# worxli/ORB_SLAM

Hardware: AMD Instinct MI355X
Metric: frames/sec ORB extract+match (640x480, 1000 kp) (higher is better)
Workload: dtype u8

## Files before the change

orb_slam_amd/csrc/orbx_extract.hip:

```cpp
#include <algorithm>
#include <type_traits>

#include "orbx_device.h"
#include "orbx_internal.h"

namespace orbx {

constexpr size_t kRetainLds = 128 * 1024;
constexpr int kRetainCellCap = 512;
constexpr int kSplitMinFrames = 16;
constexpr size_t kResizeLds = 96 * 1024;

__constant__ __attribute__((aligned(4))) int8_t c_pattern[256][4] = {
#include "orbx_pattern.inc"
};

#ifdef ORBX_FAST_PROFILE
__device__ unsigned long long g_fast_prof[16];
__device__ inline unsigned long long fp_stamp()
{
    unsigned long long t;
    asm volatile("s_memtime %0\n\ts_waitcnt lgkmcnt(0)" : "=s"(t)::"memory");
    return t;
}
#define FP_T0() unsigned long long _ft = fp_stamp()
#define FP_MARK(k)                                                                  \
    do {                                                                            \
        const unsigned long long _n = fp_stamp();                                   \
        if (threadIdx.x == 0) atomicAdd(&g_fast_prof[k], _n - _ft);                 \
        _ft = _n;                                                                   \
    } while (0)
#define FP_ADD(k, v) atomicAdd(&g_fast_prof[k], (unsigned long long)(v))
extern "C" int orbx_debug_fast_prof(unsigned long long* out)
{
    return hipMemcpyFromSymbol(out, HIP_SYMBOL(g_fast_prof), sizeof(unsigned long long) * 16) == hipSuccess ? 0 : -2;
}
#else
#define FP_T0()
#define FP_MARK(k)
#define FP_ADD(k, v)
#endif

struct ExtractArgs {
    const LevelGeom* levels;
    const CellGeom* cells;
    const ResizeCol* res_cols;
    const ResizeRow* res_rows;
    const int* umax;
    const uint8_t* frames;
    uint8_t* pyr_raw;
    uint8_t* pyr_blur;
    uint32_t* cell_lists;
    int32_t* cell_count;
    uint32_t* level_keys;
    int32_t* level_count;
    orbx_keypoint* out_kps;
    uint8_t* out_desc;
    int32_t* out_n;
    int32_t* error_flags;
    uint8_t* host_out;
    int32_t* retain_scratch;
    uint64_t* cell_keys64;
    uint64_t* level_keys64;
    int harris;
    int fp_contract;
    int nth_pivot;
    long long frame_pyr_bytes;
    int first_slot;
    int w, h;
    int nlevels, ncells, list_entries, level_entries, nfeatures;
    int fast_th, fast_th_low;
    int max_list_cap, max_level_cap;
    int l0_direct;
};

struct LevelSrc {
    const uint8_t* base;
    int stride;
};
static_assert(kEdge % 16 == 0, "the direct level 0 keeps the padded level's 16-byte alignment");
__device__ __forceinline__ LevelSrc level_src(const ExtractArgs& a, int f, int level, long long off, int stride)
{
    if (a.l0_direct && level == 0)
        return {a.frames + ((long long)(a.first_slot + f) * a.w * a.h - (long long)kEdge * a.w - kEdge), a.w};
    return {a.pyr_raw + (size_t)f * a.frame_pyr_bytes + off, stride};
}

template <class T>
__device__ __forceinline__ T cget(const T* p, int i)
{
#if defined(__HIP_DEVICE_COMPILE__)
    return ((const __attribute__((address_space(4))) T*)p)[i];
#else
    return p[i];
#endif
}

__device__ inline uint8_t sat_u8(int v) { return (uint8_t)min(max(v, 0), 255); }
__device__ inline int sat_s16(int v) { return min(max(v, -32768), 32767); }

struct RowWalk {
    int r, q, dr, dq, nq;
    __device__ RowWalk(int start, int stride, int n_q) : nq(n_q)
    {
        r = start / n_q;
        q = start - r * n_q;
        dr = stride / n_q;
        dq = stride - dr * n_q;
    }
    __device__ void next()
    {
        r += dr;
        q += dq;
        if (q >= nq) {
            q -= nq;
            r++;
        }
    }
};


template <int kBatch, typename T, typename Load>
__device__ inline void stage_to_lds(T* dst, int n, int tid, int nthr, Load load)
{
    for (int u0 = 0; u0 < n; u0 += kBatch * nthr) {
        T v[kBatch];
#pragma unroll
        for (int k = 0; k < kBatch; k++) v[k] = load(min(u0 + k * nthr + tid, n - 1));
#pragma unroll
        for (int k = 0; k < kBatch; k++) dst[min(u0 + k * nthr + tid, n - 1)] = v[k];
    }
}

constexpr int kPyrRows = 8;
constexpr int kPyr0Shift = (16 - kEdge % 16) % 16;

__global__ __launch_bounds__(256) void k_pyr_level0(ExtractArgs a, int q_lo, int nint)
{
    const int f = blockIdx.y;
    const LevelGeom L = cget(a.levels, 0);
    const int qpr = L.stride >> 4, nstrips = (L.ph + kPyrRows - 1) / kPyrRows;
    const int nbord = qpr - nint;
    int idx = blockIdx.x * blockDim.x + threadIdx.x;
    const uint8_t* src = a.frames + (size_t)(a.first_slot + f) * a.w * a.h;
    uint8_t* dst = a.pyr_raw + (size_t)f * a.frame_pyr_bytes + L.off;
    if (idx < nint * nstrips) {
        const int strip = idx / nint, q = q_lo + (idx - strip * nint), px0 = 16 * q;
        const int al = px0 - kEdge - kPyr0Shift;
        const int py_first = strip * kPyrRows;
        uint4 lo[kPyrRows], hi[kPyrRows];
#pragma unroll
        for (int rr = 0; rr < kPyrRows; rr++) {
            const int py = min(py_first + rr, L.ph - 1);
            const uint8_t* row = src + (size_t)reflect101(py - kEdge, L.h) * a.w + al;
            lo[rr] = *reinterpret_cast<const uint4*>(row);
            hi[rr] = *reinterpret_cast<const uint4*>(row + 16);
        }
#pragma unroll
        for (int rr = 0; rr < kPyrRows; rr++) {
            const uint32_t w[8] = {lo[rr].x, lo[rr].y, lo[rr].z, lo[rr].w, hi[rr].x, hi[rr].y, hi[rr].z, hi[rr].w};
            constexpr int d = kPyr0Shift >> 2, b = kPyr0Shift & 3;
            uint32_t o[4];
#pragma unroll
            for (int k = 0; k < 4; k++)
                o[k] = b ? __builtin_amdgcn_alignbyte(w[k + d + 1], w[k + d], b) : w[k + d];
            if (py_first + rr < L.ph)
                *reinterpret_cast<uint4*>(dst + (size_t)(py_first + rr) * L.stride + px0) = make_uint4(o[0], o[1], o[2], o[3]);
        }
        return;
    }
    idx -= nint * nstrips;
    if (idx >= nbord * L.ph) return;
    const int py = idx / nbord, k = idx - py * nbord;
    const int q = k < q_lo ? k : k + nint, px0 = 16 * q;
    const uint8_t* row = src + (size_t)reflect101(py - kEdge, L.h) * a.w;
    if (kEdge == 16 && a.w % 16 == 0 && a.w >= 32) {
        const int w16 = a.w >> 4;
        uint4 v = make_uint4(0, 0, 0, 0);
        if (q == 0) {
            const uint4 A = *reinterpret_cast<const uint4*>(row), B = *reinterpret_cast<const uint4*>(row + 16);
            v.x = __builtin_amdgcn_perm(B.x, A.w, 0x01020304u);
            v.y = __builtin_amdgcn_perm(A.w, A.z, 0x01020304u);
            v.z = __builtin_amdgcn_perm(A.z, A.y, 0x01020304u);
            v.w = __builtin_amdgcn_perm(A.y, A.x, 0x01020304u);
        } else if (q <= w16) {
            v = *reinterpret_cast<const uint4*>(row + 16 * (q - 1));
        } else if (q == w16 + 1) {
            const uint4 A = *reinterpret_cast<const uint4*>(row + a.w - 32), B = *reinterpret_cast<const uint4*>(row + a.w - 16);
            v.x = __builtin_amdgcn_perm(B.w, B.z, 0x03040506u);
            v.y = __builtin_amdgcn_perm(B.z, B.y, 0x03040506u);
            v.z = __builtin_amdgcn_perm(B.y, B.x, 0x03040506u);
            v.w = __builtin_amdgcn_perm(B.x, A.w, 0x03040506u);
        }
        *reinterpret_cast<uint4*>(dst + (size_t)py * L.stride + px0) = v;
        return;
    }
    uint8_t v[16];
#pragma unroll
    for (int i = 0; i < 16; i++) v[i] = px0 + i < L.pw ? row[reflect101(px0 + i - kEdge, L.w)] : 0;
    uint32_t o[4];
#pragma unroll
    for (int i = 0; i < 4; i++)
        o[i] = v[4 * i] | (uint32_t)v[4 * i + 1] << 8 | (uint32_t)v[4 * i + 2] << 16 | (uint32_t)v[4 * i + 3] << 24;
    *reinterpret_cast<uint4*>(dst + (size_t)py * L.stride + px0) = make_uint4(o[0], o[1], o[2], o[3]);
}

__device__ inline uint8_t resize_pixel(const uint8_t* prev, int pstride, const ResizeCol& c,
                                       const ResizeRow& r, bool vec)
{
    const uint8_t* r0 = prev + (size_t)r.sy0 * pstride;
    const uint8_t* r1 = prev + (size_t)r.sy1 * pstride;
    const int S0 = r0[c.sx0] * c.a0 + r0[c.sx1] * c.a1;
    const int S1 = r1[c.sx0] * c.a0 + r1[c.sx1] * c.a1;
    if (vec) {
        const int x0 = sat_s16(S0 >> 4), y0 = sat_s16(S1 >> 4);
        int v = sat_s16(((x0 * r.b0) >> 16) + ((y0 * r.b1) >> 16));
        v = sat_s16(v + 2) >> 2;
        return sat_u8(v);
    }
    return sat_u8((S0 * r.b0 + S1 * r.b1 + (1 << 21)) >> 22);
}

__global__ __launch_bounds__(256) void k_pyr_resize(ExtractArgs a, int level)
{
    const int f = blockIdx.y;
    const LevelGeom L = cget(a.levels, level);
    const LevelGeom P = cget(a.levels, level - 1);
    const int wpr = L.stride >> 2, nstrips = (L.ph + kPyrRows - 1) / kPyrRows;
    const int idx = blockIdx.x * blockDim.x + threadIdx.x;
    if (idx >= wpr * nstrips) return;
    const int strip = idx / wpr, q = idx - strip * wpr, px0 = 4 * q;
    const LevelSrc ps = level_src(a, f, level - 1, P.off, P.stride);
    const uint8_t* prev = ps.base + (size_t)kEdge * ps.stride + kEdge;
    uint8_t* dst = a.pyr_raw + (size_t)f * a.frame_pyr_bytes + L.off;
    ResizeCol c[4];
    bool vec[4], on[4];
#pragma unroll
    for (int b = 0; b < 4; b++) {
        on[b] = px0 + b < L.pw;
        const int x = on[b] ? reflect101(px0 + b - kEdge, L.w) : 0;
        c[b] = a.res_cols[L.res_col_off + x];
        vec[b] = x < L.nvec_resize;
    }
#pragma unroll
    for (int rr = 0; rr < kPyrRows; rr++) {
        const int py = min(strip * kPyrRows + rr, L.ph - 1);
        const ResizeRow r = a.res_rows[L.res_row_off + reflect101(py - kEdge, L.h)];
        uint32_t word = 0;
#pragma unroll
        for (int b = 0; b < 4; b++)
            if (on[b]) word |= (uint32_t)resize_pixel(prev, ps.stride, c[b], r, vec[b]) << (8 * b);
        if (strip * kPyrRows + rr < L.ph) *reinterpret_cast<uint32_t*>(dst + (size_t)py * L.stride + px0) = word;
    }
}

struct ResizeLevel {
    long long off, poff;
    int stride, pstride, w, h, pw, ph, ph_parent_h, nvec, span, strip_off, row_off, col_off;
    int packed;
    int plevel, ppad;
};

__global__ __launch_bounds__(256) void k_pyr_resize_lds(ExtractArgs a, ResizeLevel L, int pitch)
{
    extern __shared__ uint4 s_dyn[];
    __shared__ ResizeRow s_rows[kResRows];
    const int f = blockIdx.y, tid = threadIdx.x;
    const int py0 = blockIdx.x * kResRows, nrows = min(kResRows, L.ph - py0);
    const int nch = pitch >> 4;
    ResizeCol* s_cols = reinterpret_cast<ResizeCol*>(s_dyn + (size_t)L.span * nch);
    uint8_t* s_src = reinterpret_cast<uint8_t*>(s_dyn);
    const int lo = a.res_rows[L.strip_off + blockIdx.x].sy0;
    if (tid < nrows) s_rows[tid] = a.res_rows[L.row_off + reflect101(py0 + tid - kEdge, L.h)];
    stage_to_lds<4>(s_cols, L.w, tid, (int)blockDim.x, [&](int x) { return a.res_cols[L.col_off + x]; });
    const int nsrc = min(L.span, L.ph_parent_h - lo);
    const LevelSrc ps = level_src(a, f, L.plevel, L.poff, L.pstride);
    const uint8_t* pbase = ps.base + (size_t)(lo + kEdge) * ps.stride + (kEdge - L.ppad);
#ifndef RES_NO_STAGE
    {
        const float inv = 1.0f / (float)nch;
        stage_to_lds<8>(s_dyn, nsrc * nch, tid, (int)blockDim.x, [&](int u) {
            const int r = (int)(((float)u + 0.5f) * inv), c = u - r * nch;
            return *reinterpret_cast<const uint4*>(pbase + (size_t)r * ps.stride + 16 * c);
        });
    }
#endif
    __syncthreads();
    uint8_t* dst = a.pyr_raw + (size_t)f * a.frame_pyr_bytes + L.off + (size_t)py0 * L.stride;
#ifdef RES_NO_COMPUTE
    if (tid < 64) reinterpret_cast<uint32_t*>(dst)[tid] = s_src[tid * 7];
    return;
#endif
    const int nq = L.stride >> 2;
    const int q_lo = (kEdge + 3) >> 2, q_hi = L.packed ? max(q_lo, (kEdge + min(L.w, L.nvec)) >> 2) : q_lo;
    const int nfast = q_hi - q_lo;
    typedef unsigned short orbx_us2 __attribute__((ext_vector_type(2)));
    auto mh = [](uint32_t x, uint32_t y) {
        return (uint32_t)(((unsigned long long)(x & 0xFFFFFFu) * (unsigned long long)(y & 0xFFFFFFu)) >> 32);
    };
    for (int t = tid; t < nfast; t += blockDim.x) {
        const int q = q_lo + t, x0 = 4 * q - kEdge;
        int ca[4];
        uint32_t sel[4], wgt[4];
#pragma unroll
        for (int b = 0; b < 4; b++) {
            const ResizeCol c = s_cols[x0 + b];
            ca[b] = L.ppad + c.sx0;
            wgt[b] = (uint32_t)(16 * c.a0) | (uint32_t)(16 * c.a1) << 16;
        }
        const int qa = ca[0] & ~3, sh = ca[0] & 3;
#pragma unroll
        for (int b = 0; b < 4; b++) {
            const uint32_t r = (uint32_t)(ca[b] - ca[0]);
            sel[b] = r | 0x0C00u | (r + 1) << 16 | 0x0C000000u;
        }
        auto hrow = [&](int sy, uint32_t (&S)[4]) {
            const uint32_t* d = reinterpret_cast<const uint32_t*>(s_src + (sy - lo) * pitch + qa);
            const uint32_t d0 = d[0], d1 = d[1], d2 = d[2];
            const uint32_t w0 = __builtin_amdgcn_alignbyte(d1, d0, sh), w1 = __builtin_amdgcn_alignbyte(d2, d1, sh);
#pragma unroll
            for (int b = 0; b < 4; b++)
                S[b] = __builtin_amdgcn_udot2(__builtin_bit_cast(orbx_us2, __builtin_amdgcn_perm(w1, w0, sel[b])),
                                              __builtin_bit_cast(orbx_us2, wgt[b]), 0u, false) &
                       0x00FFFF00u;
        };
        uint32_t H0[4], H1[4];
        int c0 = -1, c1 = -1;
        uint2 nxt = reinterpret_cast<const uint2*>(s_rows)[0];
        for (int rr = 0; rr < nrows; rr++) {
            const uint2 cur = nxt;
            if (rr + 1 < nrows) nxt = reinterpret_cast<const uint2*>(s_rows)[rr + 1];
            const uint32_t w0 = __builtin_amdgcn_readfirstlane(cur.x), w1 = __builtin_amdgcn_readfirstlane(cur.y);
            const int sy0 = (int)(int16_t)(w0 & 0xFFFF), sy1 = (int)(int16_t)(w0 >> 16);
            const uint32_t B0 = (w1 & 0xFFFFu) << 8, B1 = (w1 >> 16) << 8;
            uint32_t A[4], B[4];
            if (sy0 == c1) {
#pragma unroll
                for (int b = 0; b < 4; b++) A[b] = H1[b];
            } else if (sy0 == c0) {
#pragma unroll
                for (int b = 0; b < 4; b++) A[b] = H0[b];
            } else {
                hrow(sy0, A);
            }
            if (sy1 == sy0) {
#pragma unroll
                for (int b = 0; b < 4; b++) B[b] = A[b];
            } else if (sy1 == c1) {
#pragma unroll
                for (int b = 0; b < 4; b++) B[b] = H1[b];
            } else {
                hrow(sy1, B);
            }
#pragma unroll
            for (int b = 0; b < 4; b++) {
                H0[b] = A[b];
                H1[b] = B[b];
            }
            c0 = sy0;
            c1 = sy1;
            uint32_t word = 0;
#pragma unroll
            for (int b = 0; b < 4; b++) word |= ((mh(A[b], B0) + mh(B[b], B1) + 2) >> 2) << (8 * b);
            *reinterpret_cast<uint32_t*>(dst + (size_t)rr * L.stride + 4 * q) = word;
        }
    }
    const int nslow = nq - nfast;
    for (int item = tid; item < nrows * nslow; item += blockDim.x) {
        const int rr = item / nslow, k = item - rr * nslow;
        const int q = k < q_lo ? k : k + nfast, px0 = 4 * q;
        const ResizeRow R = s_rows[rr];
        uint32_t word = 0;
#pragma unroll
        for (int b = 0; b < 4; b++) {
            if (px0 + b >= L.pw) continue;
            const int x = reflect101(px0 + b - kEdge, L.w);
            const ResizeCol c = s_cols[x];
            const uint8_t* r0 = s_src + (R.sy0 - lo) * pitch + L.ppad + c.sx0;
            const uint8_t* r1 = s_src + (R.sy1 - lo) * pitch + L.ppad + c.sx0;
            const int S0 = r0[0] * c.a0 + r0[1] * c.a1, S1 = r1[0] * c.a0 + r1[1] * c.a1;
            int v;
            if (x < L.nvec)
                v = (((S0 >> 4) * R.b0 >> 16) + ((S1 >> 4) * R.b1 >> 16) + 2) >> 2;
            else
                v = (S0 * R.b0 + S1 * R.b1 + (1 << 21)) >> 22;
            word |= (uint32_t)sat_u8(v) << (8 * b);
        }
        *reinterpret_cast<uint32_t*>(dst + (size_t)rr * L.stride + px0) = word;
    }
}

#ifndef ORBX_CASCADE_SINGLE_THREADS
#define ORBX_CASCADE_SINGLE_THREADS 1024
#endif
#ifdef ORBX_CASC_PROFILE
__device__ unsigned long long g_casc_prof[kMaxLevels][4];
#define CASC_T0() unsigned long long _ct = __builtin_readcyclecounter()
#define CASC_MARK(l, k)                                                          \
    do {                                                                         \
        const unsigned long long _n = __builtin_readcyclecounter();              \
        if (blockIdx.x == 0 && threadIdx.x == 0) g_casc_prof[l][k] += _n - _ct;  \
        _ct = _n;                                                                \
    } while (0)
extern "C" int orbx_debug_casc_prof(unsigned long long* out)
{
    return hipMemcpyFromSymbol(out, HIP_SYMBOL(g_casc_prof), sizeof(g_casc_prof)) == hipSuccess ? 0 : -2;
}
#else
#define CASC_T0()
#define CASC_MARK(l, k)
#endif
template <int T>
__global__ __launch_bounds__(T) void k_pyr_cascade(ExtractArgs a, const int4* plan, int buf_x, int tab_off,
                                                   int tab_cols)
{
    CASC_T0();
    const bool kTab = T >= 1024 && tab_off > 0;
    extern __shared__ uint4 s_dyn[];
    uint8_t* const lds = reinterpret_cast<uint8_t*>(s_dyn);
    const int band = blockIdx.x, f = blockIdx.y, tid = threadIdx.x;
    uint8_t* pyr = a.pyr_raw + (size_t)f * a.frame_pyr_bytes;
    const uint8_t* img = a.frames + (size_t)(a.first_slot + f) * a.w * a.h;
    ResizeCol* const t_cols = reinterpret_cast<ResizeCol*>(lds + tab_off);
    ResizeRow* const t_rows = reinterpret_cast<ResizeRow*>(t_cols + tab_cols);
    if (kTab) {
        int ncol = 0, nrow = 0;
        for (int l = 1; l < a.nlevels; l++) {
            const int4 pl = plan[band * a.nlevels + l];
            ncol += cget(a.levels, l).w;
            nrow += max(0, pl.w - pl.z + 1);
        }
        const int n = ncol + nrow;
        for (int u0 = 0; u0 < n; u0 += 4 * T) {
            uint2 v[4];
#pragma unroll
            for (int k = 0; k < 4; k++) {
                int e = u0 + k * T + tid;
                v[k] = make_uint2(0, 0);
                if (e >= n) continue;
                if (e < ncol) {
                    int l = 1, w;
                    while (e >= (w = cget(a.levels, l).w)) {
                        e -= w;
                        l++;
                    }
                    v[k] = *reinterpret_cast<const uint2*>(a.res_cols + cget(a.levels, l).res_col_off + e);
                } else {
                    e -= ncol;
                    int l = 1, m;
                    int4 pl = plan[band * a.nlevels + 1];
                    while (e >= (m = max(0, pl.w - pl.z + 1))) {
                        e -= m;
                        l++;
                        pl = plan[band * a.nlevels + l];
                    }
                    v[k] = *reinterpret_cast<const uint2*>(a.res_rows + cget(a.levels, l).res_row_off + pl.z + e);
                }
            }
#pragma unroll
            for (int k = 0; k < 4; k++) {
                const int e = u0 + k * T + tid;
                if (e < ncol) reinterpret_cast<uint2*>(t_cols)[e] = v[k];
                else if (e < n) reinterpret_cast<uint2*>(t_rows)[e - ncol] = v[k];
            }
        }
    }
    int sc0 = 0, sstride = 0;
    int tcol = 0, trow = 0;
    for (int l = 0; l < a.nlevels; l++) {
        const int4 pl = plan[band * a.nlevels + l];
        const LevelGeom L = cget(a.levels, l);
        const int stride = L.stride, c0 = pl.z, nrows = pl.w - pl.z + 1;
        uint8_t* dst = lds + (l & 1) * buf_x;
        if (l == 0) {
            const int n16 = a.w >> 4, n = nrows * n16;
            for (int u0 = 0; u0 < n; u0 += 4 * T) {
                uint4 v[4];
                int o[4];
#pragma unroll
                for (int k = 0; k < 4; k++) {
                    const int u = min(u0 + k * T + tid, n - 1), r = u / n16, q = u - r * n16;
                    v[k] = *reinterpret_cast<const uint4*>(img + (size_t)(c0 + r) * a.w + 16 * q);
                    o[k] = r * stride + kEdge + 16 * q;
                }
#pragma unroll
                for (int k = 0; k < 4; k++) *reinterpret_cast<uint4*>(dst + o[k]) = v[k];
            }
        } else if (nrows > 0) {
            const uint8_t* src = lds + ((l - 1) & 1) * buf_x;
            const int nw = (L.w + 3) >> 2;
            const int G = max(1, T / nw), g = tid / nw;
            for (int q = tid - min(g, G - 1) * nw; g < G && q < nw; q += T) {
                const int r_lo = g * nrows / G, r_hi = (g + 1) * nrows / G;
                const int px0 = 4 * q;
                int ca[4], a0[4], a1[4];
                bool vb[4], vec = true;
#pragma unroll
                for (int b = 0; b < 4; b++) {
                    const bool on = px0 + b < L.w;
                    const ResizeCol c = kTab ? t_cols[tcol + (on ? px0 + b : 0)] : a.res_cols[L.res_col_off + (on ? px0 + b : 0)];
                    ca[b] = kEdge + c.sx0;
                    a0[b] = on ? c.a0 : 0;
                    a1[b] = on ? c.a1 : 0;
                    vb[b] = px0 + b < L.nvec_resize;
                    vec = vec && (!on || vb[b]);
                }
                auto hrow = [&](int sy, int (&S)[4]) {
                    const uint8_t* base = src + (sy - sc0) * sstride;
#pragma unroll
                    for (int b = 0; b < 4; b++) S[b] = base[ca[b]] * a0[b] + base[ca[b] + 1] * a1[b];
                };
                int H0[4], H1[4], cs0 = -1, cs1 = -1;
                for (int r = r_lo; r < r_hi; r++) {
                    const ResizeRow rw = kTab ? t_rows[trow + r] : a.res_rows[L.res_row_off + c0 + r];
                    const int sy0 = rw.sy0, sy1 = rw.sy1, b0 = rw.b0, b1 = rw.b1;
                    int A[4], B[4];
                    if (sy0 == cs1) {
#pragma unroll
                        for (int b = 0; b < 4; b++) A[b] = H1[b];
                    } else if (sy0 == cs0) {
#pragma unroll
                        for (int b = 0; b < 4; b++) A[b] = H0[b];
                    } else {
                        hrow(sy0, A);
                    }
                    if (sy1 == sy0) {
#pragma unroll
                        for (int b = 0; b < 4; b++) B[b] = A[b];
                    } else if (sy1 == cs1) {
#pragma unroll
                        for (int b = 0; b < 4; b++) B[b] = H1[b];
                    } else {
                        hrow(sy1, B);
                    }
#pragma unroll
                    for (int b = 0; b < 4; b++) {
                        H0[b] = A[b];
                        H1[b] = B[b];
                    }
                    cs0 = sy0;
                    cs1 = sy1;
                    uint32_t word = 0;
                    if (vec) {
#pragma unroll
                        for (int b = 0; b < 4; b++) {
                            const int v = (((A[b] >> 4) * b0 >> 16) + ((B[b] >> 4) * b1 >> 16) + 2) >> 2;
                            word |= (uint32_t)min(v, 255) << (8 * b);
                        }
                    } else {
#pragma unroll
                        for (int b = 0; b < 4; b++) {
                            int v;
                            if (vb[b])
                                v = (((A[b] >> 4) * b0 >> 16) + ((B[b] >> 4) * b1 >> 16) + 2) >> 2;
                            else
                                v = (A[b] * b0 + B[b] * b1 + (1 << 21)) >> 22;
                            word |= (uint32_t)sat_u8(v) << (8 * b);
                        }
                    }
                    *reinterpret_cast<uint32_t*>(dst + r * stride + kEdge + px0) = word;
                }
            }
        }
        CASC_MARK(l, 0);
        __syncthreads();
        CASC_MARK(l, 1);
        const int tail = stride - L.pw;
        for (int i = tid; i < nrows * (2 * kEdge + tail); i += T) {
            const int r = i / (2 * kEdge + tail), k = i - r * (2 * kEdge + tail);
            uint8_t* row = dst + r * stride;
            if (k < 2 * kEdge) {
                const int px = k < kEdge ? k : L.w + k;
                row[px] = row[kEdge + reflect101(px - kEdge, L.w)];
            } else {
                row[L.pw + (k - 2 * kEdge)] = 0;
            }
        }
        __syncthreads();
        CASC_MARK(l, 2);
        {
            const int n16 = stride >> 4, nown = pl.y - pl.x;
            uint8_t* out = pyr + L.off;
            for (int i = tid; i < nown * n16; i += T) {
                const int rr = i / n16, q = i - rr * n16, r = pl.x + rr;
                *reinterpret_cast<uint4*>(out + (size_t)(kEdge + r) * stride + 16 * q) =
                    *reinterpret_cast<const uint4*>(dst + (r - c0) * stride + 16 * q);
            }
            for (int i = tid; i < 2 * kEdge * n16; i += T) {
                const int k = i / n16, q = i - k * n16;
                const int py = k < kEdge ? k : L.h + k;
                const int r = reflect101(py - kEdge, L.h);
                if (r >= pl.x && r < pl.y)
                    *reinterpret_cast<uint4*>(out + (size_t)py * stride + 16 * q) =
                        *reinterpret_cast<const uint4*>(dst + (r - c0) * stride + 16 * q);
            }
        }
        CASC_MARK(l, 3);
        if (l > 0) {
            tcol += L.w;
            trow += max(0, nrows);
        }
        sc0 = c0;
        sstride = stride;
    }
}

typedef _Float16 orbx_h2 __attribute__((ext_vector_type(2)));
typedef unsigned short orbx_u16x2 __attribute__((ext_vector_type(2)));
__device__ inline orbx_h2 h2_min3(orbx_h2 a, orbx_h2 b, orbx_h2 c)
{
    return __builtin_elementwise_minimum(__builtin_elementwise_minimum(a, b), c);
}
__device__ inline orbx_h2 h2_max3(orbx_h2 a, orbx_h2 b, orbx_h2 c)
{
    return __builtin_elementwise_maximum(__builtin_elementwise_maximum(a, b), c);
}
__device__ inline void fast_arc2(const uint8_t* t, int pa, int pb, int pitch, int& Sa, int& Sb)
{
    const int off[16] = {3 * pitch,      1 + 3 * pitch, 2 + 2 * pitch,  3 + pitch,
                         3,              3 - pitch,     2 - 2 * pitch,  1 - 3 * pitch,
                         -3 * pitch,     -1 - 3 * pitch, -2 - 2 * pitch, -3 - pitch,
                         -3,             -3 + pitch,    -2 + 2 * pitch, -1 + 3 * pitch};
    const int o = 3 * pitch + 3;
    int ba = pa - o, bb = pb - o;
    asm("" : "+v"(ba), "+v"(bb));
    const uint8_t* ta = t + ba;
    const uint8_t* tb = t + bb;
    auto pair = [&](int k) {
        orbx_u16x2 pv;
        pv.x = ta[k];
        pv.y = tb[k];
        return __builtin_bit_cast(uint32_t, pv) | 0x64006400u;
    };
    const orbx_h2 v = __builtin_bit_cast(orbx_h2, pair(o));
    orbx_h2 d[16];
#pragma unroll
    for (int k = 0; k < 16; k++) {
        const uint32_t w = pair(off[k] + o);
        d[k] = v - __builtin_bit_cast(orbx_h2, w);
    }
    orbx_h2 lo3[16], hi3[16];
#pragma unroll
    for (int k = 0; k < 16; k++) {
        lo3[k] = h2_min3(d[k], d[(k + 1) & 15], d[(k + 2) & 15]);
        hi3[k] = h2_max3(d[k], d[(k + 1) & 15], d[(k + 2) & 15]);
    }
    orbx_h2 m9[16], x9[16];
#pragma unroll
    for (int k = 0; k < 16; k++) {
        m9[k] = h2_min3(lo3[k], lo3[(k + 3) & 15], lo3[(k + 6) & 15]);
        x9[k] = h2_max3(hi3[k], hi3[(k + 3) & 15], hi3[(k + 6) & 15]);
    }
    orbx_h2 dk = h2_max3(m9[0], m9[1], m9[2]), br = h2_min3(x9[0], x9[1], x9[2]);
#pragma unroll
    for (int k = 3; k < 15; k += 2) {
        dk = h2_max3(dk, m9[k], m9[k + 1]);
        br = h2_min3(br, x9[k], x9[k + 1]);
    }
    dk = __builtin_elementwise_maximum(dk, m9[15]);
    br = __builtin_elementwise_minimum(br, x9[15]);
    const orbx_h2 r = __builtin_elementwise_maximum(dk, -br);
    Sa = (int)(float)r.x;
    Sb = (int)(float)r.y;
}

__device__ inline int byte_of(uint32_t w, int k) { return (int)((w >> (8 * k)) & 0xFF); }

typedef short orbx_s16x2 __attribute__((ext_vector_type(2)));
__device__ inline uint32_t pk_sub16(uint32_t a, uint32_t b)
{
    return __builtin_bit_cast(uint32_t, (orbx_s16x2)(__builtin_bit_cast(orbx_s16x2, a) - __builtin_bit_cast(orbx_s16x2, b)));
}
__device__ inline uint32_t pk_max16(uint32_t a, uint32_t b)
{
    return __builtin_bit_cast(uint32_t,
                              __builtin_elementwise_max(__builtin_bit_cast(orbx_s16x2, a), __builtin_bit_cast(orbx_s16x2, b)));
}
__device__ inline orbx_h2 h2_bytes(uint32_t w, uint32_t k64, uint32_t sel)
{
    return __builtin_bit_cast(orbx_h2, __builtin_amdgcn_perm(k64, w, sel));
}

constexpr int kFastWideThreads = 256;
__host__ __device__ constexpr int fast_tile_bytes(int hy_max, int pitch) { return (hy_max * pitch + 511) & ~511; }
__host__ __device__ constexpr int fast_lds_bytes(int tile_bytes) { return 2 * tile_bytes + tile_bytes / 32; }
__host__ __device__ constexpr int fast_static_lds(bool u32_entries) { return 4 * 384 * (u32_entries ? 4 : 2) + 64; }
#ifndef ORBX_FAST_LDS_TARGET
#define ORBX_FAST_LDS_TARGET (40 * 1024)
#endif
constexpr int kFastLdsTarget = ORBX_FAST_LDS_TARGET;
#ifndef ORBX_DIAG_REPEAT
// ... 940 lines not shown
        } else {
            e = a.level_keys[(size_t)f * a.level_entries + lev_loff + local];
            response = (float)(e >> 24);
        }
        y = (int)((e >> 12) & 0xFFF);
        x = (int)(e & 0xFFF);
        X = kEdge + (valid ? x : kHalfPatch + 8);
        Y = kEdge + (valid ? y : kHalfPatch + 8);
        const LevelSrc ls = level_src(a, f, level, lev_off, lev_stride);
        const uint8_t* ic = win + describe_stage_window(ls.base, (uint32_t)ls.stride, a.l0_direct && level == 0, lev_w,
                                                        lev_h, X, Y, win, hl);
        br = ic;
        wave_lds_sync();
        if (hl < kIcRows) {
            const int u = hl - kHalfPatch;
            m10 = u * ic[u];
#pragma unroll
            for (int v = 1; v <= kHalfPatch; v++) {
                const int d = __builtin_amdgcn_readlane(umax_l, v);
                if (u >= -d && u <= d) {
                    const int vp = ic[u + v * kBrPitch], vm = ic[u - v * kBrPitch];
                    m01 += v * (vp - vm);
                    m10 += u * (vp + vm);
                }
            }
        }
        m01 = half_wave_sum(m01);
        m10 = half_wave_sum(m10);
    }
    if (hl == 0) s_mom[slot] = int2{m01, m10};
    __syncthreads();
    if (wv == ((chunk + f) & (kWaves - 1)) && lane < 2 * kWaves) {
        const int2 m = s_mom[lane];
        const float ang = fast_atan2_deg((float)m.x, (float)m.y);
        const float factorPI = (float)(M_PI / 180.f);
        float s, c;
        cr_sincosf(__fmul_rn(ang, factorPI), &s, &c);
        s_trig[lane] = DescTrig{ang, s, c};
    }
    if (wave_on) describe_blur_window(win, X, Y, lev_w, lev_h, lev_nvec, hl);
    __syncthreads();
    if (!wave_on) return;
    const float angle = s_trig[slot].angle, sa = s_trig[slot].sa, ca = s_trig[slot].ca;
    uint8_t* desc = a.out_desc + ((size_t)(a.first_slot + f) * a.nfeatures + k) * 32;
    const uint8_t* lds_bytes = &s_patch[0][0];
    const float brf = (float)(int)(br - lds_bytes);
#pragma unroll
    for (int r = 0; r < 8; r++) {
        const orbx_f2 px = {(float)(int8_t)(pat[r] & 0xFF), (float)(int8_t)((pat[r] >> 16) & 0xFF)};
        const orbx_f2 py = {(float)(int8_t)((pat[r] >> 8) & 0xFF), (float)(int8_t)(pat[r] >> 24)};
        uint32_t a1, a2;
        orb_sample_addr2<kFma>(px, py, sa, ca, brf, a1, a2);
        const int t0 = lds_bytes[a1];
        const int t1 = lds_bytes[a2];
        const unsigned long long bits = __ballot(t0 < t1);
        if (valid && hl == r) {
            reinterpret_cast<uint32_t*>(desc)[r] = (uint32_t)(bits >> (32 * half));
            if (a.host_out)
                reinterpret_cast<uint32_t*>(a.host_out + 64 + (size_t)a.nfeatures * sizeof(orbx_keypoint) +
                                            (size_t)k * 32)[r] = (uint32_t)(bits >> (32 * half));
        }
    }
    if (valid && hl == 0) {
        orbx_keypoint kp;
        kp.x = (float)x;
        kp.y = (float)y;
        if (level != 0) {
            kp.x = __fmul_rn(kp.x, lev_scale);
            kp.y = __fmul_rn(kp.y, lev_scale);
        }
        kp.size = lev_psize;
        kp.angle = angle;
        kp.response = response;
        kp.octave = level;
        kp.class_id = -1;
        a.out_kps[(size_t)(a.first_slot + f) * a.nfeatures + k] = kp;
        if (a.host_out) reinterpret_cast<orbx_keypoint*>(a.host_out + 64)[k] = kp;
    }
}

__global__ __launch_bounds__(64) void k_debug_nth(const uint32_t* in, int n, int nth, uint32_t* out_glb,
                                                  uint32_t* out_lds, int* gpos, int pivot_mode)
{
    __shared__ uint32_t list[kRetainCellCap];
    __shared__ int pos[kRetainCellCap + 8];
    const int lane = threadIdx.x;
    for (int i = lane; i < n; i += 64) out_glb[i] = in[i];
    global_wave_sync();
    wave_nth_element<true>(out_glb, n, nth, gpos, pivot_mode);
    for (int i = lane; i < n; i += 64) list[i] = in[i];
    lds_wave_sync();
    wave_nth_element(list, n, nth, pos, pivot_mode);
    for (int i = lane; i < n; i += 64) out_lds[i] = list[i];
}

}

extern "C" int orbx_debug_nth_pivot(const uint32_t* entries, int n, int nth, int pivot_mode, uint32_t* out_glb,
                                    uint32_t* out_lds)
{
    using namespace orbx;
    if (!entries || !out_glb || !out_lds || n < 0 || n > kRetainCellCap || nth < 0 || nth > n ||
        (pivot_mode != 0 && pivot_mode != 1))
        return ORBX_ERR_ARG;
    uint32_t* d = nullptr;
    if (hipMalloc(&d, 4 * sizeof(uint32_t) * (n + 8)) != hipSuccess) return ORBX_ERR_NOMEM;
    int r = ORBX_OK;
    if (hipMemcpy(d, entries, sizeof(uint32_t) * n, hipMemcpyHostToDevice) != hipSuccess) r = ORBX_ERR_HIP;
    if (r == ORBX_OK) {
        hipLaunchKernelGGL(k_debug_nth, dim3(1), dim3(64), 0, 0, d, n, nth, d + (n + 8), d + 2 * (n + 8),
                           reinterpret_cast<int*>(d + 3 * (n + 8)), pivot_mode);
        if (hipDeviceSynchronize() != hipSuccess ||
            hipMemcpy(out_glb, d + (n + 8), sizeof(uint32_t) * n, hipMemcpyDeviceToHost) != hipSuccess ||
            hipMemcpy(out_lds, d + 2 * (n + 8), sizeof(uint32_t) * n, hipMemcpyDeviceToHost) != hipSuccess)
            r = ORBX_ERR_HIP;
    }
    (void)hipFree(d);
    return r;
}

extern "C" int orbx_debug_nth(const uint32_t* entries, int n, int nth, uint32_t* out_glb, uint32_t* out_lds)
{
    return orbx_debug_nth_pivot(entries, n, nth, ORBX_NTH_PIVOT_GCC48, out_glb, out_lds);
}

namespace orbx {

__global__ __launch_bounds__(64) void k_debug_describe_patch(const uint8_t* lev, int stride, int direct, LevelGeom L,
                                                             int X, int Y, uint8_t* out)
{
    __shared__ __attribute__((aligned(16))) uint8_t s_patch[2][kDescWaveBytes];
    const int lane = threadIdx.x, half = lane >> 5, hl = lane & 31;
    uint8_t* win = s_patch[half] + kWinPad;
    const int centre = describe_stage_window(lev, (uint32_t)stride, direct != 0, L.w, L.h, X, Y, win, hl);
    wave_lds_sync();
    describe_blur_window(win, X, Y, L.w, L.h, L.nvec_blur, hl);
    if (half == 0)
        for (int i = hl; i < kBrRows * kBrRows; i += 32) {
            const int r = i / kBrRows, c = i - r * kBrRows;
            out[i] = win[centre + (r - kBrR) * kBrPitch + (c - kBrR)];
        }
}

static void launch_level0(const Geometry& g, const ExtractArgs& x, int nb, hipStream_t st)
{
    const LevelGeom& L = g.levels[0];
    const int qpr = L.stride / 16;
    int q_lo = (kEdge + 15) / 16, q_hi = (L.w + kEdge + kPyr0Shift - 32) / 16;
    q_hi = std::min(q_hi, qpr - 1);
    const int nint = (g.w % 16 == 0 && q_hi >= q_lo) ? q_hi - q_lo + 1 : 0;
    if (nint == 0) q_lo = 0;
    const int items = nint * ((L.ph + kPyrRows - 1) / kPyrRows) + (qpr - nint) * L.ph;
    hipLaunchKernelGGL(k_pyr_level0, dim3((items + 255) / 256, nb), dim3(256), 0, st, x, q_lo, nint);
}

int launch_level0_slot(orbx_ctx* ctx, int slot)
{
    ExtractArgs a = {};
    a.levels = ctx->dgeom.levels;
    a.frames = ctx->frames;
    a.first_slot = slot;
    a.pyr_raw = ctx->pyr_raw + (size_t)slot * ctx->geom.frame_pyr_bytes;
    a.frame_pyr_bytes = ctx->geom.frame_pyr_bytes;
    a.w = ctx->geom.w;
    a.h = ctx->geom.h;
    launch_level0(ctx->geom, a, 1, ctx->stream);
    if (hipGetLastError() != hipSuccess) return ORBX_ERR_HIP;
    return ORBX_OK;
}

int launch_blur_slot(orbx_ctx* ctx, int slot)
{
    const int r0 = launch_level0_slot(ctx, slot);
    if (r0 != ORBX_OK) return r0;
    ExtractArgs a = {};
    a.levels = ctx->dgeom.levels;
    a.pyr_raw = ctx->pyr_raw + (size_t)slot * ctx->geom.frame_pyr_bytes;
    a.pyr_blur = ctx->pyr_blur;
    a.frame_pyr_bytes = ctx->geom.frame_pyr_bytes;
    hipLaunchKernelGGL(k_blur, dim3(ctx->blur_tiles_n, 1), dim3(kBlurItems), 0, ctx->stream, a, ctx->blur_tiles);
    if (hipGetLastError() != hipSuccess) return ORBX_ERR_HIP;
    return ORBX_OK;
}

}

extern "C" int orbx_debug_describe_patch(orbx_ctx* ctx, int slot, int level, int x, int y, uint8_t* out)
{
    using namespace orbx;
    if (!ctx || !out || slot < 0 || slot >= ctx->slots || level < 0 || level >= ctx->geom.nlevels) return ORBX_ERR_ARG;
    const LevelGeom& L = ctx->geom.levels[level];
    if (x < kEdge || x >= L.w - kEdge || y < kEdge || y >= L.h - kEdge) return ORBX_ERR_ARG;
    ctx_enter(ctx);
    uint8_t* d = nullptr;
    if (hipDeviceSynchronize() != hipSuccess) return ORBX_ERR_HIP;
    if (hipMalloc(&d, kBrRows * kBrRows) != hipSuccess) return ORBX_ERR_NOMEM;
    const bool direct = level == 0 && kEdge == 16 && ctx->geom.w % 16 == 0;
    const long long fw = ctx->geom.w, fh = ctx->geom.h;
    const uint8_t* lev = direct ? ctx->frames + ((long long)slot * fw * fh - (long long)kEdge * fw - kEdge)
                                : ctx->pyr_raw + (size_t)slot * ctx->geom.frame_pyr_bytes + L.off;
    hipLaunchKernelGGL(k_debug_describe_patch, dim3(1), dim3(64), 0, ctx->stream, lev, direct ? (int)fw : L.stride,
                       direct ? 1 : 0, L, kEdge + x, kEdge + y, d);
    int r = ORBX_OK;
    if (hipStreamSynchronize(ctx->stream) != hipSuccess ||
        hipMemcpy(out, d, kBrRows * kBrRows, hipMemcpyDeviceToHost) != hipSuccess)
        r = ORBX_ERR_HIP;
    (void)hipFree(d);
    return r;
}

extern "C" int orbx_debug_level0_direct(orbx_ctx* ctx)
{
    if (!ctx) return ORBX_ERR_ARG;
    return ctx->last_l0_direct ? 1 : 0;
}

namespace orbx {

int launch_extract(orbx_ctx* ctx, int first, int count, const MatchSpec* m)
{
    const Geometry& g = ctx->geom;
    if (count > 1 || (m && m->kind != 0 && ctx->async_match)) {
        const int r = ensure_aux_streams(ctx);
        if (r != ORBX_OK) return r;
    }
    for (int sl = first; sl < first + count && sl < (int)ctx->bow_ready.size(); sl++) ctx->bow_ready[sl] = 0;
    wait_uploads_overlap(ctx, first, count, ctx->stream);
    ExtractArgs a;
    a.levels = ctx->dgeom.levels;
    a.cells = ctx->dgeom.cells;
    a.res_cols = ctx->dgeom.res_cols;
    a.res_rows = ctx->dgeom.res_rows;
    a.umax = ctx->dgeom.umax;
    a.frames = ctx->frames;
    a.pyr_raw = ctx->pyr_raw + (size_t)first * g.frame_pyr_bytes;
    a.pyr_blur = nullptr;
    a.cell_lists = ctx->cell_lists + (size_t)first * g.list_entries;
    a.cell_count = ctx->cell_count + (size_t)first * g.cells.size();
    a.level_keys = ctx->level_keys + (size_t)first * g.level_entries;
    a.level_count = ctx->level_count + (size_t)first * g.nlevels;
    a.out_kps = ctx->out_kps;
    a.out_desc = ctx->out_desc;
    a.out_n = ctx->out_n;
    a.error_flags = ctx->error_flags;
    a.host_out = ctx->single_frame ? ctx->single_out : nullptr;
    a.retain_scratch = ctx->retain_scratch + (size_t)first * (g.list_entries + 4 * g.cells.size());
    a.harris = ctx->harris;
    a.fp_contract = ctx->fp_contract;
    a.nth_pivot = ctx->nth_pivot;
    if ((size_t)((ctx->harris ? 3 : 2) * g.max_level_cap + 8) * 4 > 160 * 1024) return ORBX_ERR_UNSUPPORTED;
    a.cell_keys64 = ctx->harris ? ctx->cell_keys64 + (size_t)first * g.list_entries : nullptr;
    a.level_keys64 = ctx->harris ? ctx->level_keys64 + (size_t)first * g.level_entries : nullptr;
    a.frame_pyr_bytes = g.frame_pyr_bytes;
    a.w = g.w;
    a.h = g.h;
    a.nlevels = g.nlevels;
    a.ncells = (int)g.cells.size();
    a.list_entries = g.list_entries;
    a.level_entries = g.level_entries;
    a.nfeatures = g.nfeatures;
    a.fast_th = min(max(g.fast_th, 0), 255);
    a.fast_th_low = 7;
    a.max_list_cap = g.max_list_cap;
    a.max_level_cap = g.max_level_cap;
    a.l0_direct = (kEdge == 16 && g.w % 16 == 0 && !(ctx->single_frame && g.cascade_bands > 0)) ? 1 : 0;
    ctx->last_l0_direct = a.l0_direct != 0;

    auto run_pyramid = [&](const ExtractArgs& x, int nb, hipStream_t st) {
        if (ctx->single_frame && g.cascade_bands > 0) {
            timer_begin(ctx, "resize", st);
            for (int rep = 0; rep < kDiagRepeat[0]; rep++) {
                {
                    int tab_off = (g.cascade_lds + 15) & ~15;
                    size_t lds = (size_t)tab_off + 8 * (size_t)(g.cascade_tab_cols + g.cascade_tab_rows);
                    if (lds > 160 * 1024) {
                        tab_off = 0;
                        lds = g.cascade_lds;
                    }
                    hipLaunchKernelGGL(k_pyr_cascade<ORBX_CASCADE_SINGLE_THREADS>, dim3(g.cascade_bands, nb),
                                       dim3(ORBX_CASCADE_SINGLE_THREADS), lds, st, x, ctx->cascade, g.cascade_buf_x,
                                       tab_off, g.cascade_tab_cols);
                }
            }
            timer_end(ctx, "resize", st);
            return;
        }
        if (!x.l0_direct) {
            timer_begin(ctx, "pyr0", st);
            launch_level0(g, x, nb, st);
            timer_end(ctx, "pyr0", st);
        }
        for (int l = 1; l < g.nlevels; l++) {
            const LevelGeom& L = g.levels[l];
            const LevelGeom& P = g.levels[l - 1];
            const int ppad = (l == 1 && x.l0_direct) ? 0 : kEdge;
            const int pitch = (ppad + P.w + 15) & ~15;
            const size_t lds = (size_t)L.res_span * pitch + (size_t)L.w * sizeof(ResizeCol);
            timer_begin(ctx, "resize", st);
            if (lds <= kResizeLds) {
                const int threads = std::min(256, ((L.stride / 4) + 63) & ~63);
                int packed = 1;
                for (int x0 = 0; x0 + 3 < L.w; x0 += 4)
                    if (g.res_cols[L.res_col_off + x0 + 3].sx0 - g.res_cols[L.res_col_off + x0].sx0 > 6) packed = 0;
                const ResizeLevel rl{L.off, P.off, L.stride, P.stride, L.w, L.h, L.pw, L.ph, P.h, L.nvec_resize,
                                     L.res_span, L.res_strip_off, L.res_row_off, L.res_col_off, packed, l - 1, ppad};
                for (int rep = 0; rep < kDiagRepeat[0]; rep++)
                    hipLaunchKernelGGL(k_pyr_resize_lds, dim3((L.ph + kResRows - 1) / kResRows, nb), dim3(threads), lds,
                                       st, x, rl, pitch);
            } else {
                const int items = (L.stride / 4) * ((L.ph + kPyrRows - 1) / kPyrRows);
                hipLaunchKernelGGL(k_pyr_resize, dim3((items + 255) / 256, nb), dim3(256), 0, st, x, l);
            }
            timer_end(ctx, "resize", st);
        }
    };
    auto run_rest = [&](const ExtractArgs& x, int nb, hipStream_t st, int parts) {
        if (parts & 1) {
        timer_begin(ctx, "fast", st);
        {
            int wmax = 0, hmax = 0;
            for (const CellGeom& c : g.cells) {
                if (!c.valid) continue;
                wmax = std::max(wmax, (15 + c.hx + 15) & ~15);
                hmax = std::max(hmax, c.hy);
            }
            const dim3 grid((int)g.cells.size(), nb);
            auto plan = [&](int P, int static_lds, int& band_rows) {
                band_rows = 0;
                const int whole = fast_tile_bytes(hmax, P);
                if (fast_lds_bytes(whole) + static_lds <= kFastLdsTarget || hmax <= 9) return whole;
                int wh = hmax;
                while (wh > 9 && fast_lds_bytes(fast_tile_bytes(wh, P)) + static_lds > kFastLdsTarget) wh--;
                const int nint = hmax - 6, bmax = wh - 8;
                const int nbands = (nint + bmax - 1) / bmax;
                band_rows = (nint + nbands - 1) / nbands;
                return fast_tile_bytes(std::min(hmax, band_rows + 8), P);
            };
            auto fast = [&](auto kern, int bytes, int band_rows, int threads) {
                const int lds = fast_lds_bytes(bytes);
                hipLaunchKernelGGL(kern, grid, dim3(threads), lds, st, x, bytes, band_rows);
            };
            int br = 0, bytes = 0;
            auto fits = [&](int P) {
                if (wmax > P) return false;
                bytes = fast_tile_bytes(hmax, P);
                return bytes <= 65536;
            };
            auto fits_banded = [&](int P) {
                if (wmax > P) return false;
                bytes = plan(P, fast_static_lds(false), br);
                return bytes <= 65536;
            };
            if (fits(96)) fast(k_fast_cells<96>, bytes, 0, 256);
            else if (fits(144)) {
                for (int rep = 0; rep < kDiagRepeat[3]; rep++) fast(k_fast_cells<144>, bytes, 0, 256);
            } else if (fits(208)) fast(k_fast_cells<208>, bytes, 0, 256);
            else if (fits_banded(336)) fast(k_fast_cells<336, kFastWideThreads, true>, bytes, br, kFastWideThreads);
            else {
                bytes = plan(wmax, fast_static_lds(true), br);
                fast(k_fast_cells<0, kFastWideThreads, true>, bytes, br, kFastWideThreads);
            }
        }
        timer_end(ctx, "fast", st);
        }
        if (parts & 2) {
        timer_begin(ctx, "retain", st);
        {
            const int ew = x.harris ? 2 : 1;
            const int cw = (ew + 1) * kRetainCellCap + 8;
            const int cwaves = 4;
            const int lw = (ew + 1) * g.max_level_cap + 8;
            const int lwaves = 1;
            const dim3 cgrid(((int)g.cells.size() + cwaves - 1) / cwaves, nb), lgrid((g.nlevels + lwaves - 1) / lwaves, nb);
            if (x.harris) {
                hipLaunchKernelGGL(k_harris_cells, dim3((int)g.cells.size(), nb), dim3(256), 0, st, x);
                hipLaunchKernelGGL(k_retain_cells<uint64_t>, cgrid, dim3(64 * cwaves), (size_t)cwaves * cw * 4, st, x,
                                   cwaves, cw);
                hipLaunchKernelGGL(k_retain_levels<uint64_t>, lgrid, dim3(64 * lwaves), (size_t)lwaves * lw * 4, st, x,
                                   lwaves, lw);
            } else {
                hipLaunchKernelGGL(k_retain_cells<uint32_t>, cgrid, dim3(64 * cwaves), (size_t)cwaves * cw * 4, st, x,
                                   cwaves, cw);
                hipLaunchKernelGGL(k_retain_levels<uint32_t>, lgrid, dim3(64 * lwaves), (size_t)lwaves * lw * 4, st, x,
                                   lwaves, lw);
            }
        }
        timer_end(ctx, "retain", st);
        }
        if (!(parts & 8)) return;
        timer_begin(ctx, "describe", st);
        const dim3 dgrid((g.nfeatures + 2 * kWaves - 1) / (2 * kWaves), xcd_frames(nb));
        for (int rep = 0; rep < kDiagRepeat[2]; rep++) {
            if (x.fp_contract)
                hipLaunchKernelGGL(k_describe<true>, dgrid, dim3(256), 0, st, x, nb);
            else
                hipLaunchKernelGGL(k_describe<false>, dgrid, dim3(256), 0, st, x, nb);
        }
        timer_end(ctx, "describe", st);
    };
    auto run = [&](const ExtractArgs& x, int nb, hipStream_t st) {
        run_pyramid(x, nb, st);
        run_rest(x, nb, st, 15);
    };
    int err = ORBX_OK;
    auto match_runs = [&](int lo, int hi, int plo, int phi, hipStream_t st) {
        if (!m || m->kind == 0) return;
        auto prev = [&](int sl) { return (sl % m->seq_len == 0) ? sl + m->seq_len - 1 : sl - 1; };
        auto take = [&](int sl) {
            const int p = prev(sl);
            return phi < 0 || (p >= plo && p < phi);
        };
        for (int s0 = lo; s0 < hi;) {
            if (!take(s0)) {
                s0++;
                continue;
            }
            int s1 = s0 + 1;
            while (s1 < hi && take(s1)) s1++;
            const int r = m->kind == 1 ? launch_match_prev(ctx, s0, s1 - s0, m->seq_len, m->window, m->nnratio,
                                                           m->check_ori, st)
                                       : launch_match_bf_prev(ctx, s0, s1 - s0, m->seq_len, m->th_low, m->nnratio, st);
            if (r != ORBX_OK) err = r;
            s0 = s1;
        }
    };
    a.first_slot = first;
    const bool async = m && m->kind != 0 && ctx->async_match && ctx->mstream;
    if (!async) {
        wait_pending_overlap(ctx, first, count, ctx->stream);
        ctx->stream_dirty = true;
    }
    if (async) {
        const int ways = std::min(ctx->split_ways, count / kSplitMinFrames);
        if (ctx->split && ways >= 2 && ctx->stream2) {
            wait_pending_overlap(ctx, first, count, ctx->stream);
            const hipStream_t S[orbx_ctx::kMaxWays] = {ctx->stream, ctx->stream2, ctx->xstreams[0], ctx->xstreams[1]};
            for (int i = 0; i < ways; i++) {
                const int lo = count * i / ways, n = count * (i + 1) / ways - lo;
                ExtractArgs b = a;
                b.first_slot = first + lo;
                b.pyr_raw += (size_t)lo * a.frame_pyr_bytes;
                b.cell_lists += (size_t)lo * a.list_entries;
                b.retain_scratch += (size_t)lo * (a.list_entries + 4 * a.ncells);
                b.cell_count += (size_t)lo * a.ncells;
                b.level_keys += (size_t)lo * a.level_entries;
                if (a.harris) {
                    b.cell_keys64 += (size_t)lo * a.list_entries;
                    b.level_keys64 += (size_t)lo * a.level_entries;
                }
                b.level_count += (size_t)lo * a.nlevels;
                if (i > 0) ORBX_HIP_CHECK(hipStreamWaitEvent(S[i], ctx->ev_part_fast[i - 1], 0));
                run_pyramid(b, n, S[i]);
                run_rest(b, n, S[i], 1);
                ORBX_HIP_CHECK(hipEventRecord(ctx->ev_part_fast[i], S[i]));
                run_rest(b, n, S[i], 14);
                ORBX_HIP_CHECK(hipEventRecord(ctx->ev_part_done[i], S[i]));
                ORBX_HIP_CHECK(hipStreamWaitEvent(ctx->mstream, ctx->ev_part_done[i], 0));
            }
        } else {
            const int r = launch_extract(ctx, first, count, nullptr);
            if (r != ORBX_OK) return r;
            ORBX_HIP_CHECK(hipEventRecord(ctx->ev_extracted, ctx->stream));
            ORBX_HIP_CHECK(hipStreamWaitEvent(ctx->mstream, ctx->ev_extracted, 0));
        }
        match_runs(first, first + count, 0, -1, ctx->mstream);
        const int q = m->seq_len;
        const int lo = (first / q) * q, hi = ((first + count + q - 1) / q) * q;
        ORBX_HIP_CHECK(push_pending(ctx, lo, hi));
        if (err != ORBX_OK) return err;
        if (hipGetLastError() != hipSuccess) return ORBX_ERR_HIP;
        return ORBX_OK;
    }
    if (ctx->split && count >= 2 * kSplitMinFrames && ctx->stream2) {
        const int n0 = count / 2, n1 = count - n0;
        ExtractArgs b = a;
        b.first_slot = first + n0;
        b.pyr_raw += (size_t)n0 * a.frame_pyr_bytes;
        b.cell_lists += (size_t)n0 * a.list_entries;
        b.retain_scratch += (size_t)n0 * (a.list_entries + 4 * a.ncells);
        b.cell_count += (size_t)n0 * a.ncells;
        b.level_keys += (size_t)n0 * a.level_entries;
        if (a.harris) {
            b.cell_keys64 += (size_t)n0 * a.list_entries;
            b.level_keys64 += (size_t)n0 * a.level_entries;
        }
        b.level_count += (size_t)n0 * a.nlevels;
        ORBX_HIP_CHECK(hipEventRecord(ctx->ev_fork, ctx->stream));
        ORBX_HIP_CHECK(hipStreamWaitEvent(ctx->stream2, ctx->ev_fork, 0));
        run(a, n0, ctx->stream);
        match_runs(first, first + n0, first, first + n0, ctx->stream);
        run(b, n1, ctx->stream2);
        match_runs(first + n0, first + count, first + n0, first + count, ctx->stream2);
        ORBX_HIP_CHECK(hipEventRecord(ctx->ev_join, ctx->stream2));
        ORBX_HIP_CHECK(hipStreamWaitEvent(ctx->stream, ctx->ev_join, 0));
        match_runs(first, first + n0, first + n0, 0x7fffffff, ctx->stream);
        match_runs(first, first + n0, -0x7fffffff, first, ctx->stream);
        match_runs(first + n0, first + count, first, first + n0, ctx->stream);
        match_runs(first + n0, first + count, first + count, 0x7fffffff, ctx->stream);
        match_runs(first + n0, first + count, -0x7fffffff, first, ctx->stream);
    } else if (ctx->single_frame && count == 1) {
        run_pyramid(a, 1, ctx->stream);
        run_rest(a, 1, ctx->stream, 1 | 2 | 8);
        match_runs(first, first + count, 0, -1, ctx->stream);
    } else {
        run(a, count, ctx->stream);
        match_runs(first, first + count, 0, -1, ctx->stream);
    }
    if (err != ORBX_OK) return err;
    if (hipGetLastError() != hipSuccess) return ORBX_ERR_HIP;
    return ORBX_OK;
}


}
```

Baseline: 284,400.

## Restructure pyramid resize kernel with sliding rows, remainder-split lanes, and border copy

Precomputes a per-row sliding descriptor flagging when the first source row must be recomputed, so the main fast path reuses horizontal sums from the previous row without branching on cached indices. Columns that leave a partial wave are split across lanes by row groups instead of leaving lanes idle. For packed levels, border columns are produced by mirroring already-written interior pixels with byte permutes rather than recomputing bilinear samples. This adds an extra barrier and host-side parameter computation, and more code paths that must stay consistent with reflect-101 semantics.

```diff
diff --git a/orb_slam_amd/csrc/orbx_extract.hip b/orb_slam_amd/csrc/orbx_extract.hip
--- a/orb_slam_amd/csrc/orbx_extract.hip
+++ b/orb_slam_amd/csrc/orbx_extract.hip
@@ -259,19 +259,28 @@
     int stride, pstride, w, h, pw, ph, ph_parent_h, nvec, span, strip_off, row_off, col_off;
     int packed;
     int plevel, ppad;
+    int nslide, rem_wave, rem_n;
 };
 
 __global__ __launch_bounds__(256) void k_pyr_resize_lds(ExtractArgs a, ResizeLevel L, int pitch)
 {
     extern __shared__ uint4 s_dyn[];
     __shared__ ResizeRow s_rows[kResRows];
+    __shared__ __attribute__((aligned(16))) uint2 s_slide[kResRows];
     const int f = blockIdx.y, tid = threadIdx.x;
     const int py0 = blockIdx.x * kResRows, nrows = min(kResRows, L.ph - py0);
     const int nch = pitch >> 4;
     ResizeCol* s_cols = reinterpret_cast<ResizeCol*>(s_dyn + (size_t)L.span * nch);
     uint8_t* s_src = reinterpret_cast<uint8_t*>(s_dyn);
     const int lo = a.res_rows[L.strip_off + blockIdx.x].sy0;
-    if (tid < nrows) s_rows[tid] = a.res_rows[L.row_off + reflect101(py0 + tid - kEdge, L.h)];
+    if (tid < nrows) {
+        const ResizeRow e = a.res_rows[L.row_off + reflect101(py0 + tid - kEdge, L.h)];
+        s_rows[tid] = e;
+        const ResizeRow p = a.res_rows[L.row_off + reflect101(py0 + max(tid, 1) - 1 - kEdge, L.h)];
+        const uint32_t first = (tid == 0 || p.sy1 != e.sy0) ? 0x1000u : 0u;
+        s_slide[tid] = make_uint2((uint32_t)(uint16_t)e.sy0 | (uint32_t)(uint16_t)e.sy1 << 16,
+                                  (uint32_t)(uint16_t)e.b0 | first | (uint32_t)(uint16_t)e.b1 << 16);
+    }
     stage_to_lds<4>(s_cols, L.w, tid, (int)blockDim.x, [&](int x) { return a.res_cols[L.col_off + x]; });
     const int nsrc = min(L.span, L.ph_parent_h - lo);
     const LevelSrc ps = level_src(a, f, L.plevel, L.poff, L.pstride);
@@ -298,7 +307,8 @@
     auto mh = [](uint32_t x, uint32_t y) {
         return (uint32_t)(((unsigned long long)(x & 0xFFFFFFu) * (unsigned long long)(y & 0xFFFFFFu)) >> 32);
     };
-    for (int t = tid; t < nfast; t += blockDim.x) {
+    auto word_rows = [&](auto uni, int t, int r0, int r1) {
+        constexpr bool kUni = decltype(uni)::value;
         const int q = q_lo + t, x0 = 4 * q - kEdge;
         int ca[4];
         uint32_t sel[4], wgt[4];
@@ -324,13 +334,42 @@
                                               __builtin_bit_cast(orbx_us2, wgt[b]), 0u, false) &
                        0x00FFFF00u;
         };
+        uint8_t* out = dst + (size_t)r0 * L.stride + 4 * q;
+        if constexpr (kUni) {
+            static_assert(kResRows % 2 == 0, "the sliding form reads s_slide in pairs");
+            uint32_t X[4], Y[4];
+            auto row = [&](const uint32_t w0, const uint32_t w1, uint32_t (&P)[4], uint32_t (&Q)[4]) {
+                const uint32_t B0 = (w1 & 0xFFFu) << 8, B1 = (w1 >> 16) << 8;
+                if (w1 & 0x1000u) {
+                    asm volatile("; first source row");
+                    hrow((int)(w0 & 0xFFFFu), Q);
+                }
+                hrow((int)(w0 >> 16), P);
+                uint32_t word = 0;
+#pragma unroll
+                for (int b = 0; b < 4; b++) word |= ((mh(Q[b], B0) + mh(P[b], B1) + 2) >> 2) << (8 * b);
+                *reinterpret_cast<uint32_t*>(out) = word;
+                out += L.stride;
+            };
+            int rr = 0;
+            uint4 e = *reinterpret_cast<const uint4*>(s_slide);
+            for (; rr + 1 < r1; rr += 2) {
+                const uint32_t a0 = __builtin_amdgcn_readfirstlane(e.x), a1 = __builtin_amdgcn_readfirstlane(e.y);
+                const uint32_t c0 = __builtin_amdgcn_readfirstlane(e.z), c1 = __builtin_amdgcn_readfirstlane(e.w);
+                e = *reinterpret_cast<const uint4*>(s_slide + min(rr + 2, kResRows - 2));
+                row(a0, a1, X, Y);
+                row(c0, c1, Y, X);
+            }
+            if (rr < r1) row(__builtin_amdgcn_readfirstlane(e.x), __builtin_amdgcn_readfirstlane(e.y), X, Y);
+            return;
+        }
+        uint2 nxt = reinterpret_cast<const uint2*>(s_rows)[r0];
         uint32_t H0[4], H1[4];
         int c0 = -1, c1 = -1;
-        uint2 nxt = reinterpret_cast<const uint2*>(s_rows)[0];
-        for (int rr = 0; rr < nrows; rr++) {
+        for (int rr = r0; rr < r1; rr++, out += L.stride) {
             const uint2 cur = nxt;
-            if (rr + 1 < nrows) nxt = reinterpret_cast<const uint2*>(s_rows)[rr + 1];
-            const uint32_t w0 = __builtin_amdgcn_readfirstlane(cur.x), w1 = __builtin_amdgcn_readfirstlane(cur.y);
+            if (rr + 1 < r1) nxt = reinterpret_cast<const uint2*>(s_rows)[rr + 1];
+            const uint32_t w0 = cur.x, w1 = cur.y;
             const int sy0 = (int)(int16_t)(w0 & 0xFFFF), sy1 = (int)(int16_t)(w0 >> 16);
             const uint32_t B0 = (w1 & 0xFFFFu) << 8, B1 = (w1 >> 16) << 8;
             uint32_t A[4], B[4];
@@ -362,13 +401,18 @@
             uint32_t word = 0;
 #pragma unroll
             for (int b = 0; b < 4; b++) word |= ((mh(A[b], B0) + mh(B[b], B1) + 2) >> 2) << (8 * b);
-            *reinterpret_cast<uint32_t*>(dst + (size_t)rr * L.stride + 4 * q) = word;
-        }
-    }
-    const int nslow = nq - nfast;
-    for (int item = tid; item < nrows * nslow; item += blockDim.x) {
-        const int rr = item / nslow, k = item - rr * nslow;
-        const int q = k < q_lo ? k : k + nfast, px0 = 4 * q;
+            *reinterpret_cast<uint32_t*>(out) = word;
+        }
+    };
+    const int rem = nfast - L.nslide;
+    for (int t = tid; t < L.nslide; t += blockDim.x) word_rows(std::true_type{}, t, 0, nrows);
+    if (rem > 0 && __builtin_amdgcn_readfirstlane(tid >> 6) == L.rem_wave) {
+        const int lane = tid & 63, g = (int)(((float)lane + 0.5f) * (1.0f / (float)rem));
+        const int r0 = g * L.rem_n;
+        if (r0 < nrows) word_rows(std::false_type{}, L.nslide + lane - g * rem, r0, min(r0 + L.rem_n, nrows));
+    }
+    auto general_word = [&](int rr, int q) {
+        const int px0 = 4 * q;
         const ResizeRow R = s_rows[rr];
         uint32_t word = 0;
 #pragma unroll
@@ -387,6 +431,37 @@
             word |= (uint32_t)sat_u8(v) << (8 * b);
         }
         *reinterpret_cast<uint32_t*>(dst + (size_t)rr * L.stride + px0) = word;
+    };
+    const int nslow = nq - nfast;
+    if (L.packed && L.w >= 2 * kEdge) {
+        const int q_in = (kEdge + L.w + 3) >> 2, ntail = q_in - q_hi;
+        for (int item = (int)blockDim.x - 1 - tid; item < kResRows * ntail; item += blockDim.x) {
+            const int rr = item % kResRows;
+            if (rr < nrows) general_word(rr, q_hi + item / kResRows);
+        }
+        __syncthreads();
+        const int ncopy = q_lo + nq - q_in;
+        for (int item = tid; item < kResRows * ncopy; item += blockDim.x) {
+            const int rr = item % kResRows, k = item / kResRows;
+            if (rr >= nrows) continue;
+            const int q = k < q_lo ? k : q_in + (k - q_lo), p0 = 4 * q;
+            const int nb = L.pw - p0;
+            uint8_t* row = dst + (size_t)rr * L.stride;
+            uint32_t word = 0;
+            if (nb > 0) {
+                const int s = (k < q_lo ? 2 * kEdge : 2 * (kEdge + L.w - 1)) - p0 - 3;
+                const uint32_t* g = reinterpret_cast<const uint32_t*>(row + (s & ~3));
+                const uint32_t v = __builtin_amdgcn_alignbyte(g[1], g[0], s & 3);
+                word = __builtin_amdgcn_perm(0u, v, 0x00010203u);
+                if (nb < 4) word &= (1u << (8 * nb)) - 1u;
+            }
+            *reinterpret_cast<uint32_t*>(row + p0) = word;
+        }
+        return;
+    }
+    for (int item = tid; item < nrows * nslow; item += blockDim.x) {
+        const int rr = item / nslow, k = item - rr * nslow;
+        general_word(rr, k < q_lo ? k : k + nfast);
     }
 }
 
@@ -1933,8 +2008,18 @@
                 int packed = 1;
                 for (int x0 = 0; x0 + 3 < L.w; x0 += 4)
                     if (g.res_cols[L.res_col_off + x0 + 3].sx0 - g.res_cols[L.res_col_off + x0].sx0 > 6) packed = 0;
+                const int q_lo = (kEdge + 3) >> 2;
+                const int nfast = packed ? std::max(q_lo, (kEdge + std::min(L.w, L.nvec_resize)) >> 2) - q_lo : 0;
+                int nslide = nfast, rem_wave = 0, rem_n = 0;
+                if (const int rem = nfast & 63; rem > 0 && rem <= 32) {
+                    nslide = nfast - rem;
+                    rem_wave = (nslide >> 6) % (threads >> 6);
+                    const int groups = 64 / rem;
+                    rem_n = (kResRows + groups - 1) / groups;
+                }
                 const ResizeLevel rl{L.off, P.off, L.stride, P.stride, L.w, L.h, L.pw, L.ph, P.h, L.nvec_resize,
-                                     L.res_span, L.res_strip_off, L.res_row_off, L.res_col_off, packed, l - 1, ppad};
+                                     L.res_span, L.res_strip_off, L.res_row_off, L.res_col_off, packed, l - 1, ppad,
+                                     nslide, rem_wave, rem_n};
                 for (int rep = 0; rep < kDiagRepeat[0]; rep++)
                     hipLaunchKernelGGL(k_pyr_resize_lds, dim3((L.ph + kResRows - 1) / kResRows, nb), dim3(threads), lds,
                                        st, x, rl, pitch);
```

Result: faster. 295,000, median of 6 (+3.7%).
